# zju3dv/EnvGS

Measured on AMD Instinct MI355X. Metric: train iters/s (fwd+bwd of the render hot path + Adam step, one 800x800 view per GPU per iter) + render Mpix/s, higher is better.
Workload: dtype f32

## Files before the change

envgs_amd/_lib.py:

```python
import ctypes
import os

import torch

HERE = os.path.dirname(os.path.abspath(__file__))
LIB_PATH = os.path.join(HERE, "libenvgs_hip.so")
_lib = None

c_void_p, c_int, c_uint32, c_size_t = ctypes.c_void_p, ctypes.c_int, ctypes.c_uint32, ctypes.c_size_t


class RasterCfg(ctypes.Structure):
    _fields_ = [("P", ctypes.c_int32), ("sh_degree", ctypes.c_int32), ("sh_coeffs", ctypes.c_int32),
                ("channels", ctypes.c_int32), ("width", ctypes.c_int32), ("height", ctypes.c_int32),
                ("bg_len", ctypes.c_int32), ("debug", ctypes.c_int32), ("scale_modifier", ctypes.c_float),
                ("tanfovx", ctypes.c_float), ("tanfovy", ctypes.c_float), ("feature_f16", ctypes.c_int32)]


class AdamTensor(ctypes.Structure):
    _fields_ = [("param", ctypes.c_void_p), ("grad", ctypes.c_void_p), ("exp_avg", ctypes.c_void_p), ("exp_avg_sq", ctypes.c_void_p),
                ("numel", ctypes.c_int64), ("lr", ctypes.c_float), ("step", ctypes.c_float)]


class RowsTensor(ctypes.Structure):
# ... 8 lines not shown
    _fields_ = ([("P", ctypes.c_int64), ("N", ctypes.c_int32), ("flags", ctypes.c_uint32)]
                + [(n, ctypes.c_float) for n in ("grad_threshold", "size_limit", "split_screen_threshold", "min_opacity", "min_gradient", "r")]
                + [(n, ctypes.c_void_p) for n in ("ga", "dn", "mr", "wa", "scal", "opac", "cls", "scan", "counters", "temp")]
                + [("temp_bytes", ctypes.c_size_t)])


class DensifyRewriteArgs(ctypes.Structure):
    _fields_ = ([("P", ctypes.c_int64), ("out_rows", ctypes.c_int64), ("n_samples", ctypes.c_int64), ("N", ctypes.c_int32), ("count", ctypes.c_int32),
                 ("ratio_n", ctypes.c_double), ("r", ctypes.c_float), ("reserved0", ctypes.c_uint32)]
                + [(n, ctypes.c_void_p) for n in ("cls", "scan", "counters", "scal", "rotation", "samples")]
                + [("tensors", ctypes.POINTER(GrowTensor))])


class TraceLists(ctypes.Structure):
    _fields_ = [("hit_lists", ctypes.c_void_p), ("hit_cnt", ctypes.c_void_p), ("n_used", ctypes.c_void_p), ("cap", ctypes.c_int32),
                ("surf_acc", ctypes.c_void_p), ("surf_cnt", ctypes.c_void_p), ("surf_off", ctypes.c_void_p),
                ("scan_temp", ctypes.c_void_p), ("scan_temp_bytes", ctypes.c_size_t), ("ray_keys", ctypes.c_void_p),
                ("ray_order", ctypes.c_void_p), ("ray_sort_temp", ctypes.c_void_p), ("ray_sort_temp_bytes", ctypes.c_size_t),
                ("records", ctypes.c_void_p),
                ("num_records", ctypes.c_uint64), ("hit_state", ctypes.c_void_p), ("entries", ctypes.c_void_p), ("pairs", ctypes.c_void_p),
                ("n_entries", ctypes.c_void_p), ("compact_rows", ctypes.c_uint64), ("row_off", ctypes.c_void_p), ("batch_rows", ctypes.c_void_p),
                ("row_blk", ctypes.c_void_p), ("sh_perm", ctypes.c_void_p), ("state_planes", ctypes.c_int32),
                ("sparse_hits", ctypes.c_void_p), ("sparse_cap", ctypes.c_uint64),
                ("defer_reduce", ctypes.c_uint32), ("reserved0", ctypes.c_uint32)]


class TraceCfg(ctypes.Structure):
    _fields_ = [("P", ctypes.c_int32), ("num_rays", ctypes.c_int32), ("sh_degree", ctypes.c_int32),
                ("sh_coeffs", ctypes.c_int32), ("max_trace_depth", ctypes.c_int32), ("start_from_first", ctypes.c_int32),
                ("has_others", ctypes.c_int32), ("bg_len", ctypes.c_int32), ("debug", ctypes.c_int32),
                ("ray_h", ctypes.c_int32), ("ray_w", ctypes.c_int32),
                ("scale_modifier", ctypes.c_float), ("specular_threshold", ctypes.c_float), ("feature_f16", ctypes.c_int32)]


class SupervisorArgs(ctypes.Structure):
    _fields_ = ([("N", ctypes.c_int64), ("P", ctypes.c_int64), ("flags", ctypes.c_uint32), ("reserved0", ctypes.c_uint32),
                 ("weight", ctypes.c_float * 5), ("reserved1", ctypes.c_float)]
                + [(n, ctypes.c_void_p) for n in ("norm_map", "surf_norm_map", "acc_map", "dpt_map", "dist_map", "env_opacity", "prior", "msk", "R", "near_far")]
                + [(n, ctypes.c_int64) for n in ("norm_map_row", "norm_map_ch", "surf_norm_map_row", "surf_norm_map_ch", "acc_map_row", "dpt_map_row",
                                                 "dist_map_row", "env_opacity_row", "prior_row", "prior_ch", "msk_row")]
                + [(n, ctypes.c_void_p) for n in ("g_norm_map", "g_surf_norm_map", "g_acc_map", "g_dist_map", "g_env_opacity", "partial")])


class SurfelInputsArgs(ctypes.Structure):
    _fields_ = ([(n, ctypes.c_int32) for n in ("P", "sh_degree", "sh_coeffs", "spec_channels")]
                + [(n, ctypes.c_void_p) for n in ("xyz", "features_dc", "features_rest", "scaling", "rotation", "opacity", "specular", "roughness", "campos",
                                                  "scales", "rotations", "opacities", "specular_act", "roughness_act", "shs", "colors", "others", "vertices",
# ... 148 lines not shown
```

envgs_amd/csrc/trace_api.hip:

```cpp
#include "trace_common.h"

#include <mutex>


namespace envgs {

constexpr int MAX_SEG = 4;

static int persistent_grid(int R, int per_cu = 8)
{
    int dev = 0, cus = 256;
    if (hipGetDevice(&dev) == hipSuccess) {
        int v = 0;
        if (hipDeviceGetAttribute(&v, hipDeviceAttributeMultiprocessorCount, dev) == hipSuccess && v > 0) cus = v;
    }
    const int want = (R + 63) / 64;
    const int cap = cus * per_cu;
    return want < cap ? (want > 0 ? want : 1) : cap;
}

static int stride_grid(int R, int per_block)
{
    const int want = (R + per_block - 1) / per_block;
    const int cap = 256 * 32;
// ... 50 lines not shown
    return true;
}

static int join_deferred(hipStream_t stream)
{
    int dev = 0;
    if (hipGetDevice(&dev) != hipSuccess || dev < 0 || dev >= 16) return 0;
    std::lock_guard<std::mutex> lk(s_mu);
    if (!s_def_pending[dev]) return 0;
    s_def_pending[dev] = false;
    return hipStreamWaitEvent(stream, s_def_done[dev], 0) == hipSuccess ? 0 : ENVGS_ERR_BAD_ARG;
}

static TraceArgs base_args(const envgs_trace_cfg *cfg, const float *nodes, const float *srec, const float *shs, const float *colors_precomp,
                           const float *others_precomp, const float *bg, const float *ray_o, const float *ray_d, uint32_t *counters)
{
    TraceArgs A = TraceArgs{};
    A.P = cfg->P; A.R = cfg->num_rays; A.D = cfg->sh_degree; A.M = cfg->sh_coeffs; A.ND = 1;
    A.start_from_first = cfg->start_from_first; A.has_others = cfg->has_others; A.bg_len = cfg->bg_len; A.spec_thr = cfg->specular_threshold;
    A.nodes = (const float4 *)nodes; A.srec = (const float4 *)srec; A.shs = shs; A.colors = colors_precomp; A.others = others_precomp;
    A.bg = bg; A.ray_o = ray_o; A.ray_d = ray_d; A.counter = counters;
    A.mod = cfg->scale_modifier; A.f16 = cfg->feature_f16; A.exp = debug_switch(ENVGS_DBG_TRACE);
    return A;
}

static unsigned sparse_capacity(const envgs_trace_lists *L)
{
    return (unsigned)(L->sparse_cap > 0xFFFFFFF0ull ? 0xFFFFFFF0ull : L->sparse_cap);
}

extern "C" {

size_t envgs_trace_ray_sort_temp_bytes(int32_t num_rays) { return ray_sort_temp_bytes(num_rays); }

int envgs_trace_ray_order(int32_t num_rays, const float *ray_o, const float *ray_d, const float *nodes, int32_t P, uint64_t *pairs,
                          uint32_t *order, void *temp, size_t temp_bytes, void *stream)
{
    if (num_rays < 0 || P < 0) return ENVGS_ERR_BAD_ARG;
    if (num_rays == 0) return 0;
    if (!ray_o || !ray_d || !pairs || !order || !temp || (P > 0 && !nodes)) return ENVGS_ERR_BAD_ARG;
    return launch_ray_sort(num_rays, ray_o, ray_d, (const float4 *)nodes, P, pairs, order, temp, temp_bytes, (hipStream_t)stream);
}

int envgs_trace_forward(const envgs_trace_cfg *cfg, const float *nodes, const float *ray_o, const float *ray_d,
                        const float *means3D, const float *scales, const float *rotations, const float *opacities,
                        const float *shs, const float *colors_precomp, const float *others_precomp, const float *bg,
// ... 133 lines not shown
            }
            {
                ProfScope p2(K_TRACE_SORT, st);
                const dim3 g(stride_grid(rays_seg, 4)), b(256);
                if (S.shp) hipLaunchKernelGGL((sort_composite_fwd<4, false, true>), g, b, 0, st, S);
                else hipLaunchKernelGGL((sort_composite_fwd<4, false, false>), g, b, 0, st, S);
                if (S.cap > 256) {
                    const dim3 gl(min(stride_grid(rays_seg, 256), 512));
                    if (S.cap <= 512) { if (S.shp) hipLaunchKernelGGL((sort_composite_fwd<8, true, true>), gl, b, 0, st, S); else hipLaunchKernelGGL((sort_composite_fwd<8, true, false>), gl, b, 0, st, S); }
                    else { if (S.shp) hipLaunchKernelGGL((sort_composite_fwd<16, true, true>), gl, b, 0, st, S); else hipLaunchKernelGGL((sort_composite_fwd<16, true, false>), gl, b, 0, st, S); }
                }
            }
            ENVGS_CHECK_LAUNCH(dcfg, st);
            {
                ProfScope p8(K_TRACE_REGISTER, st);
                const dim3 gr(stride_grid(rays_seg, 64)), br(64 * RH_W);
                if (S.pairs && S.cap <= 256) hipLaunchKernelGGL(register_hits<true>, gr, br, 0, st, S);
                else hipLaunchKernelGGL(register_hits<false>, gr, br, 0, st, S);
            }
            ENVGS_CHECK_LAUNCH(dcfg, st);
        }
        for (int i = 1; i < nseg; i++)
            if (hipEventRecord(ev_join[i], aux[i]) != hipSuccess || hipStreamWaitEvent(stream, ev_join[i], 0) != hipSuccess) return ENVGS_ERR_BAD_ARG;
        hipLaunchKernelGGL(unpack_surfel_acc, dim3((cfg->P + 255) / 256), dim3(256), 0, stream, cfg->P, A.wfrac, A.surf_acc, L->surf_cnt, wet,
                           counters);
        ENVGS_CHECK_LAUNCH(dcfg, stream);
        {
            const int rc = launch_scan(L->surf_cnt, L->surf_off, cfg->P * NCOPY, L->scan_temp, L->scan_temp_bytes, stream);
            if (rc) return rc;
        }
        A.only_overflow = 1;
    } else {
        const int rcp = launch_prepare(stream);
        if (rcp) return rcp;
        ENVGS_CHECK_LAUNCH(dcfg, stream);
    }
    { ProfScope p4(K_TRACE_KBUF_FWD, stream); hipLaunchKernelGGL(trace_fwd, dim3(persistent_grid(cfg->num_rays)), dim3(64), 0, stream, A, rh, rw); }
    ENVGS_CHECK_LAUNCH(dcfg, stream);
    return 0;
}

int envgs_trace_backward(const envgs_trace_cfg *cfg, const float *nodes, const float *ray_o, const float *ray_d,
                         const float *means3D, const float *scales, const float *rotations, const float *opacities,
                         const float *shs, const float *colors_precomp, const float *others_precomp, const float *bg,
                         const float *srec, uint32_t *counters, const float *rgb, const float *dpt, const float *acc,
                         const float *norm, const float *aux, const float *final_T, const float *dL_drgb, const float *dL_ddpt,
                         const float *dL_dacc, const float *dL_dnorm, const float *dL_daux, float *geo_rec, float *dmeans3D,
                         float *dgrads3D, float *dscales, float *drots, float *dopacities, float *dshs, float *dcolors,
// ... 31 lines not shown
    A.geo_rec = geo_rec; A.dshs = dshs; A.dcolors = dcolors; A.dothers = dothers; A.dray_o = dray_o; A.dray_d = dray_d;
    if (A.exp & (8 | 16 | 512 | 2048 | 4096 | 8192)) return ENVGS_ERR_BAD_ARG;
    int rh, rw; ray_layout(cfg, &rh, &rw);
    bool deferred = false, have_records = false;
    int def_dev = 0;
    {
        ProfScope prof_(K_TRACE_BWD, stream);
        if (lists_wanted(cfg, L) && !lists_usable_bwd(cfg, L)) return ENVGS_ERR_BAD_ARG;
        if (lists_usable_bwd(cfg, L)) {
            A.hits = (uint2 *)L->hit_lists; A.hit_cnt = L->hit_cnt; A.n_used = L->n_used; A.cap = L->cap;
            if (L->ray_keys && L->ray_order && L->ray_sort_temp && !(A.exp & 64)) A.order = L->ray_order + cfg->num_rays;
            if (L->records && L->num_records > 0 && L->surf_cnt && L->surf_off && L->hit_state && L->entries && L->pairs && L->n_entries) {
                A.surf_cnt = L->surf_cnt; A.surf_off = L->surf_off; A.records = L->records; A.num_records = L->num_records;
                A.state = (float4 *)L->hit_state; A.entries = (unsigned long long *)L->entries; A.pairs = L->pairs; A.n_entries = L->n_entries;
                if (L->compact_rows > 0) {
                    if (!L->row_off || !L->batch_rows) return ENVGS_ERR_BAD_ARG;
                    A.row_off = L->row_off; A.batch_rows = (const uint2 *)L->batch_rows;
                }
                A.state_plane = L->compact_rows > 0 ? (size_t)L->compact_rows : (size_t)cfg->num_rays * (size_t)L->cap;
                {
                    ProfScope p5(K_TRACE_LIST_BWD, stream);
                    const bool rgb_only = dL_drgb && !dL_ddpt && !dL_dacc && !dL_dnorm && !dL_daux;
                    if (L->state_planes == 1 && !rgb_only) return ENVGS_ERR_BAD_ARG;
                    const dim3 g(stride_grid((cfg->num_rays + 63) / 64, 1));
                    if (rgb_only) hipLaunchKernelGGL((batch_surfel_bwd<true, false>), g, dim3(64), 0, stream, A);
                    else if (cfg->has_others) hipLaunchKernelGGL((batch_surfel_bwd<false, true>), g, dim3(64), 0, stream, A);
                    else hipLaunchKernelGGL((batch_surfel_bwd<false, false>), g, dim3(64), 0, stream, A);
                    if (L->sparse_hits && L->sparse_cap > 0) {
                        A.sparse = (uint4 *)L->sparse_hits;
                        A.sparse_cap = sparse_capacity(L);
                        hipLaunchKernelGGL(sparse_hits_bwd, dim3(2048), dim3(256), 0, stream, A, rgb_only ? 1 : 0);
                    }
                }
                have_records = true;
                if ((dflags & ENVGS_TRACE_DEFER) && aux_objects(&def_dev)) deferred = true;
                else if (!accumulate) { ProfScope p7(K_TRACE_REDUCE, stream); hipLaunchKernelGGL(reduce_surfel_records, dim3(stride_grid(cfg->P, 16)), dim3(256), 0, stream, A); }
            } else {
                if (!(L->surf_cnt && L->surf_off && L->hit_state && L->entries && L->pairs && L->n_entries) || (L->records == nullptr && L->num_records > 0))
                    return ENVGS_ERR_BAD_ARG;
            }
            A.only_overflow = 1;
        }
        if (accumulate && join_deferred(stream)) return ENVGS_ERR_BAD_ARG;
        { ProfScope p6(K_TRACE_KBUF_BWD, stream); hipLaunchKernelGGL(trace_bwd, dim3(persistent_grid(cfg->num_rays)), dim3(64), 0, stream, A, rh, rw); }
    }
    ENVGS_CHECK_LAUNCH(dcfg, stream);
    if ((dflags & ENVGS_TRACE_DEFER) && !deferred && aux_objects(&def_dev)) deferred = true;
// ... 31 lines not shown
```

envgs_amd/csrc/trace_common.h:

```cpp
#ifndef ENVGS_TRACE_COMMON_H
#define ENVGS_TRACE_COMMON_H

#include "common.h"
#include "prof.h"

#include <cstdlib>
#include <cstring>

#include "../../include/envgs_trace.h"

namespace envgs {

constexpr int KBUF = 16;
constexpr int STACK = 64;
constexpr int NCOPY = 8;
constexpr int MAX_ROUNDS = 256;
constexpr float UV_MAX = 3.0f;
constexpr int MID = ENVGS_MID_CHANNELS;
constexpr int SREC = ENVGS_SREC_STRIDE;
constexpr int NODE = ENVGS_NODE_STRIDE;

constexpr float kC0 = 0.28209479177387814f;
constexpr float kC1 = 0.4886025119029199f;
static __device__ __constant__ float tC2[5] = {1.0925484305920792f, -1.0925484305920792f, 0.31539156525252005f,
// ... 114 lines not shown
    const unsigned *surf_off;
    float *records;
    unsigned long long num_records;
    const unsigned *order;
    int exp;
    int only_overflow;
    int batch0, batch1;
    uint4 *sparse;
    unsigned sparse_cap;
    int sparse_max;
    int reduce_adds;
    int seg;
    unsigned long long *entries;
    unsigned *pairs;
    int *n_entries;
    unsigned *long_list;
    float4 *state;
    size_t state_plane;
    int colour_state;
    unsigned *batch_cnt;
    const unsigned *row_off;
    const uint2 *batch_rows;
    const void *shp;
};

struct KBuf {
    float t[KBUF];
    int id[KBUF];
    int n;
    __device__ __forceinline__ void reset() {
#pragma unroll
        for (int i = 0; i < KBUF; i++) { t[i] = 3.0e38f; id[i] = 0x7fffffff; }
        n = 0;
    }
    __device__ __forceinline__ void insert(float ct, int cid) {
#pragma unroll
        for (int i = 0; i < KBUF; i++) {
            const bool before = (ct < t[i]) || (ct == t[i] && cid < id[i]);
            const float tt = before ? t[i] : ct; const int ii = before ? id[i] : cid;
            t[i] = before ? ct : t[i]; id[i] = before ? cid : id[i];
            ct = tt; cid = ii;
        }
        n = n < KBUF ? n + 1 : KBUF;
    }
};

// ... 408 lines not shown
struct ForwardPrepare {
    ZeroBatch zero; int zero_blocks;
    int P, rec_blocks; float mod; const float *means, *scales, *rots, *opac; float *srec;
    int perm_blocks, nb, f16; const void *shs; void *shp;
};
__global__ void __launch_bounds__(256) forward_prepare(const ForwardPrepare F);
__global__ void __launch_bounds__(64) trace_fwd(const TraceArgs A, const int ray_h, const int ray_w);
__global__ void __launch_bounds__(64) trace_bwd(const TraceArgs A, const int ray_h, const int ray_w);
__global__ void __launch_bounds__(256, 8)
collect_hits_coop(const TraceArgs A, const float4 *__restrict__ nodes, const float4 *__restrict__ nodes4, const float4 *__restrict__ srec);

template <int EMAX, bool LONG, bool QSH> __global__ void __launch_bounds__(256) sort_composite_fwd(const TraceArgs A);
extern template __global__ void __launch_bounds__(256) sort_composite_fwd<4, false, false>(const TraceArgs A);
extern template __global__ void __launch_bounds__(256) sort_composite_fwd<8, true, false>(const TraceArgs A);
extern template __global__ void __launch_bounds__(256) sort_composite_fwd<16, true, false>(const TraceArgs A);
extern template __global__ void __launch_bounds__(256) sort_composite_fwd<4, false, true>(const TraceArgs A);
extern template __global__ void __launch_bounds__(256) sort_composite_fwd<8, true, true>(const TraceArgs A);
extern template __global__ void __launch_bounds__(256) sort_composite_fwd<16, true, true>(const TraceArgs A);
template <bool CACHED> __global__ void __launch_bounds__(64 * RH_W) register_hits(const TraceArgs A);
__global__ void __launch_bounds__(256) row_scan_blocks(unsigned *__restrict__ blk, int n, unsigned *rows_used, unsigned *seg_base);
__global__ void __launch_bounds__(256) row_offsets(const TraceArgs A, const unsigned *__restrict__ blk, unsigned *__restrict__ row_off, uint2 *__restrict__ batch_rows,
                                                   const unsigned *__restrict__ seg_base, unsigned long long limit);
__global__ void __launch_bounds__(256) unpack_surfel_acc(int P, int wfrac, const unsigned long long *__restrict__ acc, unsigned *__restrict__ cnt,
                                                         float *__restrict__ wet, unsigned *ray_counter);
__global__ void __launch_bounds__(256) sparse_hits_bwd(const TraceArgs A, const int rgbo);
template <bool RGBO, bool OTH> __global__ void __attribute__((amdgpu_waves_per_eu(ENVGS_BSB_WAVES, ENVGS_BSB_WAVES))) __launch_bounds__(64) batch_surfel_bwd(const TraceArgs A);
extern template __global__ void __attribute__((amdgpu_waves_per_eu(ENVGS_BSB_WAVES, ENVGS_BSB_WAVES))) __launch_bounds__(64) batch_surfel_bwd<false, false>(const TraceArgs A);
extern template __global__ void __attribute__((amdgpu_waves_per_eu(ENVGS_BSB_WAVES, ENVGS_BSB_WAVES))) __launch_bounds__(64) batch_surfel_bwd<false, true>(const TraceArgs A);
extern template __global__ void __attribute__((amdgpu_waves_per_eu(ENVGS_BSB_WAVES, ENVGS_BSB_WAVES))) __launch_bounds__(64) batch_surfel_bwd<true, false>(const TraceArgs A);
__global__ void __launch_bounds__(256) reduce_surfel_records(const TraceArgs A);
__global__ void __launch_bounds__(256) finish_surfel_grads(int P, const float *__restrict__ rots, const float *__restrict__ geo_rec,
                                                           float *__restrict__ dmeans, float *__restrict__ dscales, float *__restrict__ dopac,
                                                           float *__restrict__ drots, float *__restrict__ dgrads3D);

}
#endif
```

envgs_amd/csrc/trace_lists.hip:

```cpp
#include "trace_common.h"

#ifndef ENVGS_SCF_KO
#define ENVGS_SCF_KO 0
#endif
namespace envgs {

template <int S>
__device__ __forceinline__ unsigned xlane(unsigned v)
{
    if constexpr (S == 1) return (unsigned)__builtin_amdgcn_update_dpp(0, (int)v, 0xB1, 0xf, 0xf, true);
    else if constexpr (S == 2) return (unsigned)__builtin_amdgcn_update_dpp(0, (int)v, 0x4E, 0xf, 0xf, true);
    else if constexpr (S == 32) {
        const envgs_u2 r = __builtin_amdgcn_permlane32_swap(v, v, false, false);
        return (threadIdx.x & 32) ? r.x : r.y;
    } else return (unsigned)__builtin_amdgcn_ds_swizzle((int)v, 0x1F | (S << 10));
}

template <int E, int SIZE, int STRIDE>
__device__ __forceinline__ void bitonic_layer(unsigned long long (&k)[E], const int lane)
{
    if constexpr (STRIDE >= 64) {
        constexpr int SE = STRIDE / 64;
#pragma unroll
        for (int e = 0; e < E; e++)
// ... 628 lines not shown
    const int slot_end = min(A.R, A.batch1 * 64);
    const int slot = A.batch0 * 64 + (int)blockIdx.x * 256 + (int)threadIdx.x;
    const int lane = threadIdx.x & 63, batch = slot >> 6;
    if (batch >= A.batch1) return;
    const unsigned cnt = rows_of_slot(A, slot, slot_end);
    const float incl = wave_scan_add((float)cnt);
    const unsigned long long row0 = base + (unsigned long long)blk[batch];
    const unsigned long long row = row0 + (unsigned long long)((unsigned)incl - cnt);
    const bool fits = row + cnt <= limit;
    if (slot < slot_end) {
        row_off[slot] = (unsigned)(fits ? row : 0ull);
        if (!fits && cnt > 0u) {
            A.hit_cnt[ray_of(A, slot)] = A.cap + 1;
            atomicAdd(A.counter + 21, 1u);
        }
    }
    const unsigned tot = (unsigned)wave_bcast(incl, 63);
    if (lane == 0) {
        const unsigned long long end = row0 + tot < limit ? row0 + tot : limit;
        batch_rows[batch] = make_uint2((unsigned)(row0 < limit ? row0 : limit), (unsigned)(end > row0 ? end - row0 : 0ull));
    }
}

__global__ void __launch_bounds__(256)
unpack_surfel_acc(int P, int wfrac, const unsigned long long *__restrict__ acc, unsigned *__restrict__ cnt, float *__restrict__ wet, unsigned *ray_counter)
{
    const int i = blockIdx.x * 256 + threadIdx.x;
    if (i == 0 && ray_counter) *ray_counter = 0u;
    if (i >= P) return;
    unsigned long long wsum = 0;
#pragma unroll
    for (int c = 0; c < NCOPY; c++) {
        const unsigned long long a = acc[(size_t)i * NCOPY + c];
        cnt[(size_t)i * NCOPY + c] = (unsigned)(a & 0xFFFFFFull);
        wsum += a >> 24;
    }
    const float w = (float)((double)wsum / (double)(1ull << wfrac));
    if (w != 0.0f) wet[i] += w;
}


template __global__ void sort_composite_fwd<4, false, false>(const TraceArgs A);
template __global__ void sort_composite_fwd<8, true, false>(const TraceArgs A);
template __global__ void sort_composite_fwd<16, true, false>(const TraceArgs A);
template __global__ void sort_composite_fwd<4, false, true>(const TraceArgs A);
template __global__ void sort_composite_fwd<8, true, true>(const TraceArgs A);
template __global__ void sort_composite_fwd<16, true, true>(const TraceArgs A);

}
```

envgs_amd/csrc/trace_surfel_bwd.hip:

```cpp
#include "trace_common.h"

namespace envgs {

#define ENVGS_LDS_FENCE() do { __builtin_amdgcn_s_waitcnt(0xc07f); __builtin_amdgcn_sched_barrier(0); } while (0)
#ifndef ENVGS_BS_GROUP
#define ENVGS_BS_GROUP 15
#endif
constexpr int BS_GROUP = ENVGS_BS_GROUP;
static_assert(BS_GROUP <= 16, "stage() assigns four lanes per entry");
#ifndef ENVGS_BSB_KO
#define ENVGS_BSB_KO 0
#endif

typedef float f32x4 __attribute__((ext_vector_type(4)));
constexpr int BT_PITCH = 96;
constexpr int RECW = 64;
template <bool RGBO, bool OTH>
__global__ void __attribute__((amdgpu_waves_per_eu(ENVGS_BSB_WAVES, ENVGS_BSB_WAVES))) __launch_bounds__(64)
batch_surfel_bwd(const TraceArgs A)
{
    static_assert(!(RGBO && OTH), "the colour-only form never touches `others`");
    __shared__ float4 sdat[2][BS_GROUP][16];
    __shared__ unsigned long long sdesc[2][BS_GROUP];
    __shared__ unsigned short kmat[2][BS_GROUP][64];
    __shared__ unsigned spb[2][BS_GROUP];
    __shared__ unsigned scn[2][BS_GROUP];
    __shared__ float btile[16][BT_PITCH];
    __shared__ float2 sox[2][BS_GROUP];
    const int lane = threadIdx.x;
    const int nb = (A.D + 1) * (A.D + 1);
    const int nbatch = (A.R + 63) >> 6;
    for (int batch = blockIdx.x; batch < nbatch; batch += gridDim.x) {
        const int base = batch << 6;
        const int copy = batch & (NCOPY - 1);
        const int r = ray_of(A, base + lane);
        const bool valid = r < A.R && A.hit_cnt[r < A.R ? r : 0] <= A.cap;
        const int rr = r < A.R ? r : 0;
        float basis[16], Box, Boy, Boz, Bdx, Bdy, Bdz, gR0, gR1, gR2, gD, gA, gN0, gN1, gN2, gX0, gX1, Fsum;
        {
            BwdRay B;
            bwd_load_ray(A, rr, B);
#pragma unroll
            for (int k = 0; k < 16; k++) basis[k] = 0.f;
            sh_basis(A.D, B.ux, B.uy, B.uz, basis);
            if (A.M == 0) basis[0] = kC0;
            if (!(B.il > 0.0f && B.il < 3.0e38f)) {
#pragma unroll
                for (int k = 0; k < 16; k++) basis[k] = 0.f;
            }
            Box = B.ox; Boy = B.oy; Boz = B.oz; Bdx = B.dx; Bdy = B.dy; Bdz = B.dz;
            gR0 = B.gR0; gR1 = B.gR1; gR2 = B.gR2;
            if constexpr (RGBO) { gD = gA = gN0 = gN1 = gN2 = gX0 = gX1 = 0.f; }
            else { gD = B.gD; gA = B.gA; gN0 = B.gN0; gN1 = B.gN1; gN2 = B.gN2; gX0 = B.gX0; gX1 = B.gX1; }
            Fsum = bwd_final_dot(B);
        }
// ... 497 lines not shown
```

envgs_amd/tracing.py:

```python
from typing import NamedTuple

import torch
from torch import nn

from . import _lib


class SurfelTracingSettings(NamedTuple):
    image_height: int
    image_width: int
    tanfovx: float
    tanfovy: float
    bg: torch.Tensor
    scale_modifier: float
    viewmatrix: torch.Tensor
    projmatrix: torch.Tensor
    sh_degree: int
    campos: torch.Tensor
    prefiltered: bool
    debug: bool
    max_trace_depth: int
    specular_threshold: float


# ... 123 lines not shown
    if n * item <= (32 << 20):
        return torch.empty(shape, dtype=dtype, device=dev)
    k = max(n - 1, 1).bit_length() - 1
    for q in (5, 6, 7, 8):
        if (q << k) >> 2 >= n:
            return torch.empty((q << k) >> 2, dtype=dtype, device=dev)[:n].view(shape)
    raise AssertionError


def _carve_i32(dev, sizes):
    offs, total = {}, 0
    for k, n in sizes.items():
        offs[k] = total
        total += ((int(n) + 63) // 64) * 64
    buf = torch.empty(max(total, 64), dtype=torch.int32, device=dev)
    out = {k: buf[o:o + int(sizes[k])] for k, o in offs.items()}
    out["_i32_block"] = buf
    return out


SPARSE = {"mode": "auto", "below": 6.0, "cap": None, "poison": None}
QUAD_SH = {"on": True}
KEEP_LISTS = {"on": False}


_DEFERRED = {"pending": False, "keep": None, "dev": None}


def join_deferred_gradients():
    if not _DEFERRED["pending"]:
        return
    dev = _DEFERRED["dev"]
    with torch.cuda.device(dev):
        _lib.check(_lib.load().envgs_trace_backward_join(_stream(dev)), "envgs_trace_backward_join")
    _DEFERRED.update(pending=False, keep=None, dev=None)


class _DeferBarrier(torch.autograd.Function):

    @staticmethod
    def forward(ctx, *ts):
        return tuple(t.view_as(t) for t in ts)

    @staticmethod
    def backward(ctx, *gs):
        join_deferred_gradients()
# ... 48 lines not shown
    from .raster import _featc
    shs = _featc(shs); colors_precomp = _featc(colors_precomp); others_precomp = _f32c(others_precomp)
    f16 = any(t is not None and t.dtype == torch.float16 for t in (shs, colors_precomp))
    bg = _f32c(settings.bg).reshape(-1).to(dev)
    cfg = _cfg(settings, P, R, shs, others_precomp, start_from_first, lead, f16)
    ND = cfg.max_trace_depth + 1
    f32 = dict(dtype=torch.float32, device=dev)
    srec = torch.empty(max(P, 1), 16, **f32)
    counters = torch.empty(96, dtype=torch.int32, device=dev)
    rgb = torch.empty(R, 3, **f32); dpt = torch.empty(R, 1, **f32); acc = torch.empty(R, 1, **f32)
    norm = torch.empty(R, 3, **f32); dist = torch.empty(R, 1, **f32); aux = torch.empty(R, 2, **f32)
    mid = torch.empty(R, 16 * ND, **f32); wet = torch.empty(P, 1, **f32); final_T = torch.empty(R, **f32)
    cap = caps.next_cap(dev) if (use_lists and ND == 1 and P > 0 and R > 0) else 0
    rows = 0
    lists = None
    keep = {}
    if cap:
        i32 = dict(dtype=torch.int32, device=dev)
        sb = lib.envgs_raster_scan_temp_bytes(NCOPY * P)
        rb = lib.envgs_trace_ray_sort_temp_bytes(R)
        nbatch = (R + 63) // 64
        keep = _carve_i32(dev, dict(hit_cnt=R, n_used=R, surf_acc=2 * P * NCOPY, surf_cnt=P * NCOPY,
                                    surf_off=P * NCOPY, scan_temp=(max(sb, 1) + 3) // 4, ray_keys=2 * R, ray_order=2 * R, ray_sort_temp=(max(rb, 1) + 3) // 4,
                                    n_entries=2 * nbatch, row_off=R, batch_rows=2 * nbatch, row_blk=nbatch + 16))
        keep["n_entries"] = keep["n_entries"].view(nbatch, 2)
        keep["hit_lists"] = _scratch((R, cap, 2), torch.int32, dev)
        srt = SORT_RAYS["on"]
        if shs is not None and shs.shape[1] == 16 and QUAD_SH["on"]:
            keep["sh_perm"] = torch.empty(P, 48, dtype=shs.dtype, device=dev)
        if need_grad:
            colour_only = bool(getattr(caps, "colour_only", False))
            sw = 4 if colour_only else (10 if others_precomp is not None else 8)
            if COMPACT["on"] and srt:
                rows = caps.next_rows(R, cap)
                keep.update(hit_state=_scratch((rows, sw), torch.float32, dev), entries=_scratch((rows,), torch.int64, dev), pairs=_scratch((rows,), torch.int32, dev))
            else:
                keep.update(hit_state=_scratch((R, cap, sw), torch.float32, dev), entries=_scratch((nbatch, 64 * cap), torch.int64, dev),
                            pairs=_scratch((nbatch, 64 * cap), torch.int32, dev))
        sparse = SPARSE["mode"] == "on" or (SPARSE["mode"] == "auto" and caps.hits_per_entry is not None and caps.hits_per_entry < SPARSE["below"])
        if "hit_state" in keep and sparse:
            n_rows = rows if rows else R * cap
            keep["sparse_hits"] = _scratch((max(4096, n_rows), 4), torch.int32, dev)
            if SPARSE.get("poison") is not None:
                keep["sparse_hits"].fill_(int(SPARSE["poison"]))
        sparse_cap = 0
        if "sparse_hits" in keep:
            sparse_cap = keep["sparse_hits"].shape[0] if SPARSE.get("cap") is None else min(int(SPARSE["cap"]), keep["sparse_hits"].shape[0])
        lists = _lib.TraceLists(keep["hit_lists"].data_ptr(), keep["hit_cnt"].data_ptr(), keep["n_used"].data_ptr(), cap,
                                keep["surf_acc"].data_ptr(), keep["surf_cnt"].data_ptr(), keep["surf_off"].data_ptr(),
                                keep["scan_temp"].data_ptr(), sb, keep["ray_keys"].data_ptr() if srt else None,
                                keep["ray_order"].data_ptr() if srt else None, keep["ray_sort_temp"].data_ptr() if srt else None, rb, None, 0,
                                *[(keep[k].data_ptr() if k in keep else None) for k in ("hit_state", "entries", "pairs")],
                                keep["n_entries"].data_ptr() if "hit_state" in keep else None, rows,
                                *[(keep[k].data_ptr() if (k in keep and rows) else None) for k in ("row_off", "batch_rows", "row_blk")],
                                keep["sh_perm"].data_ptr() if "sh_perm" in keep else None, 0,
                                keep["sparse_hits"].data_ptr() if "sparse_hits" in keep else None, sparse_cap)
        if "hit_state" in keep and getattr(caps, "colour_only", False):
            lists.state_planes = 1
            keep["colour_only"] = True
        if "hit_state" in keep and getattr(caps, "defer_reduce", False):
            keep["defer_reduce"] = True
    p = _lib.ptr
    _lib.check(lib.envgs_trace_forward(cfg, p(nodes), p(ro), p(rd), p(means3D), p(scales), p(rotations), p(opacities), p(shs),
                                       p(colors_precomp), p(others_precomp), p(bg), p(srec), p(counters), p(rgb), p(dpt), p(acc),
                                       p(norm), p(dist), p(aux), p(mid), p(wet), p(final_T), lists, _stream(dev)), "envgs_trace_forward")
    LAST_STATS.update(P=P, R=R, caps=caps, rows=rows, counters=counters, n_entries=(keep.get("n_entries") if "hit_state" in keep else None), cap=cap,
                      lists=((keep["hit_lists"], keep["n_used"], keep["hit_cnt"]) if (cap and KEEP_LISTS["on"]) else None),
                      records=(dict(sparse_hits=keep.get("sparse_hits"), sparse_cap=sparse_cap, entries=keep["entries"], pairs=keep["pairs"],
                                    n_entries=keep["n_entries"], batch_rows=(keep["batch_rows"].view(-1, 2) if rows else None),
                                    ray_order=(keep["ray_order"][R:] if SORT_RAYS["on"] else None), surf_cnt=keep["surf_cnt"], surf_off=keep["surf_off"])
                               if (cap and KEEP_LISTS["on"] and "hit_state" in keep) else None))
    if cap:
        if "hit_state" in keep and not KEEP_LISTS["on"]:
            keep.pop("hit_lists")
            lists.hit_lists = None
        caps.publish(counters, dev, rays=R)
        if "hit_state" in keep:
            keep["n_rec_host"], keep["n_rec_claim"] = caps.pinned_word()
            keep["n_rec_host"].copy_(keep["surf_off"].view(-1)[NCOPY * P - 1:NCOPY * P], non_blocking=True)
            keep["n_rec_event"] = torch.cuda.Event(); keep["n_rec_event"].record(torch.cuda.current_stream(dev))
    saved = dict(cfg=cfg, nodes=nodes, ro=ro, rd=rd, means3D=means3D, scales=scales, rotations=rotations, opacities=opacities,
                 shs=shs, colors_precomp=colors_precomp, others=others_precomp, bg=bg, srec=srec, counters=counters,
                 rgb=(rgb if ND == 1 else mid[:, 13:16].contiguous()),
                 dpt=dpt, acc=acc, norm=norm, aux=aux, final_T=final_T, lead=lead, lists=lists, keep=keep, cap=cap)
    outs = (rgb.reshape(lead + (3,)), dpt.reshape(lead + (1,)), acc.reshape(lead + (1,)), norm.reshape(lead + (3,)),
            dist.reshape(lead + (1,)), aux.reshape(lead + (2,)), mid.reshape(lead + (16 * ND,)), wet)
    return outs, saved


class _BounceChain:

    def __init__(self):
        self.acc = None
# ... 397 lines not shown
```

include/envgs_raster.h:

```cpp
#ifndef ENVGS_RASTER_H
#define ENVGS_RASTER_H

#include <stddef.h>
#include <stdint.h>

#ifdef __cplusplus
extern "C" {
#endif

#if defined(__GNUC__)
#define ENVGS_API __attribute__((visibility("default")))
#else
#define ENVGS_API
#endif

#define ENVGS_TILE 16
#define ENVGS_GEOM_STRIDE 16
#define ENVGS_GRAD_STRIDE 32

typedef enum envgs_status {
    ENVGS_OK = 0,
    ENVGS_ERR_BAD_ARG = -1,
    ENVGS_ERR_TEMP_TOO_SMALL = -2
} envgs_status;
// ... 41 lines not shown
                          const uint32_t *point_list, const uint32_t *ranges,
                          const float *final_T, const int32_t *n_contrib, const uint8_t *contrib_mask ,
                          const float *dL_dcolor, const float *dL_dallmap,
                          const float *means3D, const float *scales, const float *rotations,
                          const float *shs, const uint8_t *clamped, const float *transmat_precomp,
                          const int32_t *radii,
                          const float *viewmatrix, const float *projmatrix, const float *campos,
                          float *grad_rec,
                          float *dmeans3D, float *dmeans2D, float *dscales, float *drots,
                          float *dshs, float *dcolors, float *dopacities, float *dtransmat_precomp,
                          void *stream);

ENVGS_API void envgs_prof_enable(int on);
ENVGS_API void envgs_prof_select(uint64_t kernel_mask);
ENVGS_API int envgs_prof_read(int kernel_id, double *total_ms, int *launches);
ENVGS_API const char *envgs_prof_kernel_name(int kernel_id);

#define ENVGS_DBG_TRACE 0
#define ENVGS_DBG_SEGMENTS 1
#define ENVGS_DBG_COLLECT_WGS 2
#define ENVGS_DBG_RASTER_EXACT 3
#define ENVGS_DBG_RAYKEY 4
#define ENVGS_DBG_SPARSE 5
#define ENVGS_DBG_COUNT 6
ENVGS_API void envgs_debug_set(int32_t which, int32_t value);
ENVGS_API int32_t envgs_debug_get(int32_t which);

#ifdef __cplusplus
}
#endif
#endif
```

include/envgs_trace.h:

```cpp
#ifndef ENVGS_TRACE_H
#define ENVGS_TRACE_H

#include <stddef.h>
#include <stdint.h>

#include "envgs_raster.h"

#ifdef __cplusplus
extern "C" {
#endif

#define ENVGS_NODE_STRIDE 16
#define ENVGS_SREC_STRIDE 16
#define ENVGS_GEOREC_STRIDE 16
#define ENVGS_MID_CHANNELS 16
#define ENVGS_WIDE_EMPTY ((int32_t)0x80000000)

typedef struct envgs_trace_cfg {
    int32_t P;
    int32_t num_rays;
    int32_t sh_degree;
    int32_t sh_coeffs;
    int32_t max_trace_depth;
    int32_t start_from_first;
// ... 16 lines not shown
    uint32_t *surf_off;
    void *scan_temp;
    size_t scan_temp_bytes;
    uint32_t *ray_keys;
    uint32_t *ray_order;
    void *ray_sort_temp;
    size_t ray_sort_temp_bytes;
    float *records;
    uint64_t num_records;
    float *hit_state;
    uint64_t *entries;
    uint32_t *pairs;
    int32_t *n_entries;
    uint64_t compact_rows;
    uint32_t *row_off;
    uint32_t *batch_rows;
    uint32_t *row_blk;
    void *sh_perm;
    int32_t state_planes;
    uint32_t *sparse_hits;
    uint64_t sparse_cap;
    uint32_t defer_reduce;
    uint32_t reserved0;
} envgs_trace_lists;
#define ENVGS_TRACE_DEFER 1u
#define ENVGS_TRACE_ACCUMULATE 2u
#define ENVGS_TRACE_NO_FINISH 4u

ENVGS_API size_t envgs_bvh_temp_bytes(int32_t P);
ENVGS_API size_t envgs_bvh_node_floats(int32_t P);

ENVGS_API int envgs_bvh_build(int32_t P, const float *vertices, const float *opacities, float *nodes, void *temp, size_t temp_bytes,
                              int32_t debug, void *stream);

ENVGS_API int envgs_bvh_refit(int32_t P, const float *vertices, const float *opacities, const float *nodes_prev, float *nodes, void *temp,
                              size_t temp_bytes, int32_t debug, void *stream);

ENVGS_API int envgs_bvh_quality(int32_t P, const float *nodes, float *out2, void *stream);

ENVGS_API size_t envgs_trace_ray_sort_temp_bytes(int32_t num_rays);
ENVGS_API int envgs_trace_ray_order(int32_t num_rays, const float *ray_o, const float *ray_d, const float *nodes, int32_t P,
                                    uint64_t *pairs, uint32_t *order, void *temp, size_t temp_bytes, void *stream);
ENVGS_API int envgs_trace_forward(const envgs_trace_cfg *cfg, const float *nodes,
                                  const float *ray_o, const float *ray_d,
                                  const float *means3D, const float *scales, const float *rotations, const float *opacities,
                                  const float *shs, const float *colors_precomp, const float *others_precomp, const float *bg,
                                  float *srec, uint32_t *counters,
// ... 24 lines not shown
```

Baseline: 136.2.

## Schedule surfel backward batches in descending-cost order for load balance

Adds a single-block pass, folded into the unpack_surfel_acc launch, that bins 64-ray batches by entry count into 32 cost classes. It writes a permutation ordering the heaviest batches first. The tracer backward then launches one workgroup per batch in that order instead of a strided persistent grid, aiming to cut tail imbalance across CUs. The cost is an extra serial one-block pass on the stream, a larger grid, and the loss of the strided coherence ordering.

```diff
diff --git a/envgs_amd/_lib.py b/envgs_amd/_lib.py
--- a/envgs_amd/_lib.py
+++ b/envgs_amd/_lib.py
@@ -54,7 +54,7 @@
                 ("n_entries", ctypes.c_void_p), ("compact_rows", ctypes.c_uint64), ("row_off", ctypes.c_void_p), ("batch_rows", ctypes.c_void_p),
                 ("row_blk", ctypes.c_void_p), ("sh_perm", ctypes.c_void_p), ("state_planes", ctypes.c_int32),
                 ("sparse_hits", ctypes.c_void_p), ("sparse_cap", ctypes.c_uint64),
-                ("defer_reduce", ctypes.c_uint32), ("reserved0", ctypes.c_uint32)]
+                ("defer_reduce", ctypes.c_uint32), ("reserved0", ctypes.c_uint32), ("bwd_order", ctypes.c_void_p)]
 
 
 class TraceCfg(ctypes.Structure):
diff --git a/envgs_amd/csrc/trace_api.hip b/envgs_amd/csrc/trace_api.hip
--- a/envgs_amd/csrc/trace_api.hip
+++ b/envgs_amd/csrc/trace_api.hip
@@ -96,6 +96,12 @@
     A.bg = bg; A.ray_o = ray_o; A.ray_d = ray_d; A.counter = counters;
     A.mod = cfg->scale_modifier; A.f16 = cfg->feature_f16; A.exp = debug_switch(ENVGS_DBG_TRACE);
     return A;
+}
+
+static int bwd_order_classes()
+{
+    const int k = debug_switch(ENVGS_DBG_BALANCE) >> 8;
+    return k > 0 ? k : ENVGS_BWD_ORDER_CLASSES;
 }
 
 static unsigned sparse_capacity(const envgs_trace_lists *L)
@@ -275,8 +281,9 @@
         }
         for (int i = 1; i < nseg; i++)
             if (hipEventRecord(ev_join[i], aux[i]) != hipSuccess || hipStreamWaitEvent(stream, ev_join[i], 0) != hipSuccess) return ENVGS_ERR_BAD_ARG;
-        hipLaunchKernelGGL(unpack_surfel_acc, dim3((cfg->P + 255) / 256), dim3(256), 0, stream, cfg->P, A.wfrac, A.surf_acc, L->surf_cnt, wet,
-                           counters);
+        unsigned *bwd_order = (L->bwd_order && L->n_entries && L->entries && L->pairs && L->hit_state) ? L->bwd_order : nullptr;
+        hipLaunchKernelGGL(unpack_surfel_acc, dim3((cfg->P + 255) / 256 + (bwd_order ? 1 : 0)), dim3(256), 0, stream, cfg->P, A.wfrac, A.surf_acc, L->surf_cnt, wet,
+                           counters, (const int *)L->n_entries, nbatch_all, bwd_order, bwd_order_classes());
         ENVGS_CHECK_LAUNCH(dcfg, stream);
         {
             const int rc = launch_scan(L->surf_cnt, L->surf_off, cfg->P * NCOPY, L->scan_temp, L->scan_temp_bytes, stream);
@@ -354,7 +361,9 @@
                     ProfScope p5(K_TRACE_LIST_BWD, stream);
                     const bool rgb_only = dL_drgb && !dL_ddpt && !dL_dacc && !dL_dnorm && !dL_daux;
                     if (L->state_planes == 1 && !rgb_only) return ENVGS_ERR_BAD_ARG;
-                    const dim3 g(stride_grid((cfg->num_rays + 63) / 64, 1));
+                    const bool by_cost = L->bwd_order && !(debug_switch(ENVGS_DBG_BALANCE) & 1);
+                    A.bwd_order = by_cost ? L->bwd_order : nullptr;
+                    const dim3 g(by_cost ? (cfg->num_rays + 63) / 64 : stride_grid((cfg->num_rays + 63) / 64, 1));
                     if (rgb_only) hipLaunchKernelGGL((batch_surfel_bwd<true, false>), g, dim3(64), 0, stream, A);
                     else if (cfg->has_others) hipLaunchKernelGGL((batch_surfel_bwd<false, true>), g, dim3(64), 0, stream, A);
                     else hipLaunchKernelGGL((batch_surfel_bwd<false, false>), g, dim3(64), 0, stream, A);
diff --git a/envgs_amd/csrc/trace_common.h b/envgs_amd/csrc/trace_common.h
--- a/envgs_amd/csrc/trace_common.h
+++ b/envgs_amd/csrc/trace_common.h
@@ -160,6 +160,7 @@
     const unsigned *row_off;
     const uint2 *batch_rows;
     const void *shp;
+    const unsigned *bwd_order;
 };
 
 struct KBuf {
@@ -614,7 +615,8 @@
 __global__ void __launch_bounds__(256) row_offsets(const TraceArgs A, const unsigned *__restrict__ blk, unsigned *__restrict__ row_off, uint2 *__restrict__ batch_rows,
                                                    const unsigned *__restrict__ seg_base, unsigned long long limit);
 __global__ void __launch_bounds__(256) unpack_surfel_acc(int P, int wfrac, const unsigned long long *__restrict__ acc, unsigned *__restrict__ cnt,
-                                                         float *__restrict__ wet, unsigned *ray_counter);
+                                                         float *__restrict__ wet, unsigned *ray_counter, const int *__restrict__ n_entries, int nbatch,
+                                                         unsigned *__restrict__ bwd_order, int order_classes);
 __global__ void __launch_bounds__(256) sparse_hits_bwd(const TraceArgs A, const int rgbo);
 template <bool RGBO, bool OTH> __global__ void __attribute__((amdgpu_waves_per_eu(ENVGS_BSB_WAVES, ENVGS_BSB_WAVES))) __launch_bounds__(64) batch_surfel_bwd(const TraceArgs A);
 extern template __global__ void __attribute__((amdgpu_waves_per_eu(ENVGS_BSB_WAVES, ENVGS_BSB_WAVES))) __launch_bounds__(64) batch_surfel_bwd<false, false>(const TraceArgs A);
diff --git a/envgs_amd/csrc/trace_lists.hip b/envgs_amd/csrc/trace_lists.hip
--- a/envgs_amd/csrc/trace_lists.hip
+++ b/envgs_amd/csrc/trace_lists.hip
@@ -674,10 +674,79 @@
     }
 }
 
+constexpr int ORDER_MAX_CLASSES = 1024;
+constexpr int ORDER_SEGS = 4;
+__device__ __forceinline__ int order_count(const int *__restrict__ n_entries, int b)
+{
+    const int c = n_entries[2 * b] + n_entries[2 * b + 1];
+    return c < 0 ? 0 : (c > (1 << 20) ? (1 << 20) : c);
+}
+__device__ __forceinline__ int order_bin(int cnt, int maxc, int K)
+{
+    cnt = cnt > maxc ? maxc : cnt;
+    return K - 1 - (int)(((unsigned)cnt * (unsigned)K) / ((unsigned)maxc + 1u));
+}
+__device__ void build_bwd_order(const int *__restrict__ n_entries, const int nbatch, unsigned *__restrict__ order, int K)
+{
+    __shared__ unsigned s_off[ORDER_MAX_CLASSES * ORDER_SEGS];
+    __shared__ int s_max;
+    K = K < 1 ? 1 : (K > ORDER_MAX_CLASSES ? ORDER_MAX_CLASSES : K);
+    const int tid = threadIdx.x, lane = tid & 63, wave = tid >> 6;
+    const int seglen = (((nbatch + ORDER_SEGS - 1) / ORDER_SEGS) + 63) & ~63;
+    if (tid == 0) s_max = 0;
+    for (int i = tid; i < K * ORDER_SEGS; i += 256) s_off[i] = 0u;
+    __syncthreads();
+    int m = 0;
+#pragma unroll 8
+    for (int b = tid; b < nbatch; b += 256) m = max(m, order_count(n_entries, b));
+    if (m > 0) atomicMax(&s_max, m);
+    __syncthreads();
+    const int maxc = s_max;
+#pragma unroll 8
+    for (int b = tid; b < nbatch; b += 256) atomicAdd(&s_off[order_bin(order_count(n_entries, b), maxc, K) * ORDER_SEGS + b / seglen], 1u);
+    __syncthreads();
+    if (wave == 0) {
+        unsigned carry = 0u;
+        for (int k0 = 0; k0 < K * ORDER_SEGS; k0 += 64) {
+            const unsigned v = s_off[k0 + lane];
+            unsigned incl = v;
+#pragma unroll
+            for (int d = 1; d < 64; d <<= 1) { const unsigned o = __shfl_up(incl, d); if (lane >= d) incl += o; }
+            s_off[k0 + lane] = carry + incl - v;
+            carry += __shfl(incl, 63);
+        }
+    }
+    __syncthreads();
+    int nbits = 0;
+    while ((1 << nbits) < K) nbits++;
+    const int seg0 = wave * seglen, seg1 = min(seg0 + seglen, nbatch);
+    int next = seg0 + lane < seg1 ? order_count(n_entries, seg0 + lane) : 0;
+    for (int b0 = seg0; b0 < seg1; b0 += 64) {
+        const int b = b0 + lane;
+        const bool act = b < seg1;
+        const int cnt = next;
+        next = b + 64 < seg1 ? order_count(n_entries, b + 64) : 0;
+        const int bin = act ? order_bin(cnt, maxc, K) : 0;
+        unsigned long long mask = __ballot(act);
+        for (int bit = 0; bit < nbits; bit++) {
+            const bool one = (bin >> bit) & 1;
+            const unsigned long long bb = __ballot(act && one);
+            mask &= one ? bb : ~bb;
+        }
+        const int rank = __popcll(mask & ((1ull << lane) - 1ull));
+        unsigned first = 0u;
+        if (act && rank == 0) first = atomicAdd(&s_off[bin * ORDER_SEGS + wave], (unsigned)__popcll(mask));
+        first = __shfl(first, act ? __ffsll((long long)mask) - 1 : lane);
+        if (act && first + (unsigned)rank < (unsigned)nbatch) order[first + (unsigned)rank] = (unsigned)b;
+    }
+}
+
 __global__ void __launch_bounds__(256)
-unpack_surfel_acc(int P, int wfrac, const unsigned long long *__restrict__ acc, unsigned *__restrict__ cnt, float *__restrict__ wet, unsigned *ray_counter)
-{
-    const int i = blockIdx.x * 256 + threadIdx.x;
+unpack_surfel_acc(int P, int wfrac, const unsigned long long *__restrict__ acc, unsigned *__restrict__ cnt, float *__restrict__ wet, unsigned *ray_counter,
+                  const int *__restrict__ n_entries, int nbatch, unsigned *__restrict__ bwd_order, int order_classes)
+{
+    if (bwd_order && blockIdx.x == 0) { build_bwd_order(n_entries, nbatch, bwd_order, order_classes); return; }
+    const int i = (int)(blockIdx.x - (bwd_order ? 1u : 0u)) * 256 + threadIdx.x;
     if (i == 0 && ray_counter) *ray_counter = 0u;
     if (i >= P) return;
     unsigned long long wsum = 0;
diff --git a/envgs_amd/csrc/trace_surfel_bwd.hip b/envgs_amd/csrc/trace_surfel_bwd.hip
--- a/envgs_amd/csrc/trace_surfel_bwd.hip
+++ b/envgs_amd/csrc/trace_surfel_bwd.hip
@@ -30,7 +30,9 @@
     const int lane = threadIdx.x;
     const int nb = (A.D + 1) * (A.D + 1);
     const int nbatch = (A.R + 63) >> 6;
-    for (int batch = blockIdx.x; batch < nbatch; batch += gridDim.x) {
+    for (int slot = blockIdx.x; slot < nbatch; slot += gridDim.x) {
+        const int batch = A.bwd_order ? (int)A.bwd_order[slot] : slot;
+        if ((unsigned)batch >= (unsigned)nbatch) continue;
         const int base = batch << 6;
         const int copy = batch & (NCOPY - 1);
         const int r = ray_of(A, base + lane);
diff --git a/envgs_amd/tracing.py b/envgs_amd/tracing.py
--- a/envgs_amd/tracing.py
+++ b/envgs_amd/tracing.py
@@ -169,6 +169,12 @@
 SPARSE = {"mode": "auto", "below": 6.0, "cap": None, "poison": None}
 QUAD_SH = {"on": True}
 KEEP_LISTS = {"on": False}
+BWD_ORDER = {"on": True}
+BWD_ORDER_CLASSES = 32
+
+
+def bwd_order_class(counts, classes=BWD_ORDER_CLASSES):
+    return (counts * int(classes)) // (int(counts.max()) + 1)
 
 
 _DEFERRED = {"pending": False, "keep": None, "dev": None}
@@ -263,7 +269,7 @@
         nbatch = (R + 63) // 64
         keep = _carve_i32(dev, dict(hit_cnt=R, n_used=R, surf_acc=2 * P * NCOPY, surf_cnt=P * NCOPY,
                                     surf_off=P * NCOPY, scan_temp=(max(sb, 1) + 3) // 4, ray_keys=2 * R, ray_order=2 * R, ray_sort_temp=(max(rb, 1) + 3) // 4,
-                                    n_entries=2 * nbatch, row_off=R, batch_rows=2 * nbatch, row_blk=nbatch + 16))
+                                    n_entries=2 * nbatch, row_off=R, batch_rows=2 * nbatch, row_blk=nbatch + 16, bwd_order=nbatch))
         keep["n_entries"] = keep["n_entries"].view(nbatch, 2)
         keep["hit_lists"] = _scratch((R, cap, 2), torch.int32, dev)
         srt = SORT_RAYS["on"]
@@ -296,6 +302,8 @@
                                 *[(keep[k].data_ptr() if (k in keep and rows) else None) for k in ("row_off", "batch_rows", "row_blk")],
                                 keep["sh_perm"].data_ptr() if "sh_perm" in keep else None, 0,
                                 keep["sparse_hits"].data_ptr() if "sparse_hits" in keep else None, sparse_cap)
+        if "hit_state" in keep and BWD_ORDER["on"]:
+            lists.bwd_order = keep["bwd_order"].data_ptr()
         if "hit_state" in keep and getattr(caps, "colour_only", False):
             lists.state_planes = 1
             keep["colour_only"] = True
@@ -309,7 +317,8 @@
                       lists=((keep["hit_lists"], keep["n_used"], keep["hit_cnt"]) if (cap and KEEP_LISTS["on"]) else None),
                       records=(dict(sparse_hits=keep.get("sparse_hits"), sparse_cap=sparse_cap, entries=keep["entries"], pairs=keep["pairs"],
                                     n_entries=keep["n_entries"], batch_rows=(keep["batch_rows"].view(-1, 2) if rows else None),
-                                    ray_order=(keep["ray_order"][R:] if SORT_RAYS["on"] else None), surf_cnt=keep["surf_cnt"], surf_off=keep["surf_off"])
+                                    ray_order=(keep["ray_order"][R:] if SORT_RAYS["on"] else None), surf_cnt=keep["surf_cnt"], surf_off=keep["surf_off"],
+                                    bwd_order=(keep["bwd_order"] if BWD_ORDER["on"] else None))
                                if (cap and KEEP_LISTS["on"] and "hit_state" in keep) else None))
     if cap:
         if "hit_state" in keep and not KEEP_LISTS["on"]:
diff --git a/include/envgs_raster.h b/include/envgs_raster.h
--- a/include/envgs_raster.h
+++ b/include/envgs_raster.h
@@ -87,7 +87,8 @@
 #define ENVGS_DBG_RASTER_EXACT 3
 #define ENVGS_DBG_RAYKEY 4
 #define ENVGS_DBG_SPARSE 5
-#define ENVGS_DBG_COUNT 6
+#define ENVGS_DBG_BALANCE 6
+#define ENVGS_DBG_COUNT 7
 ENVGS_API void envgs_debug_set(int32_t which, int32_t value);
 ENVGS_API int32_t envgs_debug_get(int32_t which);
 
diff --git a/include/envgs_trace.h b/include/envgs_trace.h
--- a/include/envgs_trace.h
+++ b/include/envgs_trace.h
@@ -62,7 +62,9 @@
     uint64_t sparse_cap;
     uint32_t defer_reduce;
     uint32_t reserved0;
+    uint32_t *bwd_order;
 } envgs_trace_lists;
+#define ENVGS_BWD_ORDER_CLASSES 32
 #define ENVGS_TRACE_DEFER 1u
 #define ENVGS_TRACE_ACCUMULATE 2u
 #define ENVGS_TRACE_NO_FINISH 4u
diff --git a/profiles/balance_profile.py b/profiles/balance_profile.py
--- /dev/null
+++ b/profiles/balance_profile.py
@@ -0,0 +1,92 @@
+import argparse
+import importlib
+import importlib.util
+import os
+import sys
+
+HERE = os.path.dirname(os.path.abspath(__file__))
+sys.path[:] = [os.path.dirname(HERE)] + [p for p in sys.path if os.path.abspath(p or ".") != HERE]
+
+import numpy as np
+import torch
+
+_spec = importlib.util.spec_from_file_location("sched_model", os.path.join(HERE, "sched_model.py"))
+sched_model = importlib.util.module_from_spec(_spec)
+_spec.loader.exec_module(sched_model)
+from envgs_amd import envgs_step, raster, synth, tracing
+
+
+def main():
+    ap = argparse.ArgumentParser()
+    ap.add_argument("--out", required=True)
+    ap.add_argument("--save-counts", default=None, help="directory for the per-view count arrays (.npy)")
+    ap.add_argument("--gaussians", type=int, default=300000)
+    ap.add_argument("--env-gaussians", type=int, default=163840)
+    ap.add_argument("--res", type=int, default=800)
+    a = ap.parse_args()
+    dev = torch.device("cuda:0")
+    P, H, W, C = a.gaussians, a.res, a.res, 5
+    g = synth.base_gaussians(P, seed=0, device=dev)
+    ge = synth.env_gaussians(a.env_gaussians, seed=1, device=dev)
+    cams = [synth.orbit_camera(v, n_views=8, H=H, W=W, fx=1111.1 * W / 800.0, device=dev) for v in range(8)]
+    names = ["means3D", "shs", "opacities", "scales", "rotations"]
+    params = {k: g[k].clone().requires_grad_(True) for k in names}
+    params["specular"] = g["specular"].repeat(1, C - 4).contiguous().clone().requires_grad_(True)
+    params["roughness"] = g["roughness"].clone().requires_grad_(True)
+    env = {k: ge[k].clone().requires_grad_(True) for k in names}
+    pkg = importlib.import_module("diff_surfel_rasterization_wet_ch05")
+    import diff_surfel_tracing as tpkg
+    envgs_step.FUSED["on"] = True
+    tracer = tpkg.SurfelTracer()
+    bg = torch.zeros(3, device=dev)
+    sh_degree = torch.tensor([3], device=dev)
+    lines = []
+    out = lambda s="": (lines.append(s), print(s, flush=True))
+    out("balance of the coarse work, %d base / %d environment surfels, %dx%d, the eight bench views" % (P, a.env_gaussians, H, W))
+    out()
+    out("== tracer backward: entries per 64-ray batch of the environment trace ==")
+    for v, cam in enumerate(cams):
+        for _ in range(2):
+            envgs_step.envgs_forward(pkg, tpkg, tracer, cam, synth.get_rays(cam), params, env, bg, bg, sh_degree)
+        torch.cuda.synchronize()
+        tracing.join_deferred_gradients()
+        ne = tracing.LAST_STATS["n_entries"].cpu().numpy().astype(np.int64)
+        if a.save_counts:
+            os.makedirs(a.save_counts, exist_ok=True)
+            np.save(os.path.join(a.save_counts, "n_entries_view%d.npy" % v), ne)
+        out("view %d" % v)
+        out(sched_model.format_report(sched_model.report(ne)).rstrip("\n"))
+    out()
+    out("== raster: per-tile work summed over the eight XCD bands of xcd_tile() ==")
+    out("(instances = entries of the tile's list; contributing = entries some pixel of the tile blended; passes = (8x8 quadrant, splat) passes of R7)")
+    for v, cam in enumerate(cams):
+        st = pkg.GaussianRasterizationSettings(image_height=H, image_width=W, tanfovx=cam.tanfovx, tanfovy=cam.tanfovy, bg=torch.zeros(C, device=dev),
+                                               scale_modifier=1.0, viewmatrix=cam.world_view_transform, projmatrix=cam.full_proj_transform,
+                                               sh_degree=sh_degree, campos=cam.camera_center, prefiltered=False, debug=False)
+        with torch.no_grad():
+            _, sv = raster.rasterize_forward(C, g["means3D"], None, torch.zeros(P, C, device=dev), g["opacities"], g["scales"], g["rotations"], None, st)
+        rg = sv["ranges"].view(-1, 2).long().cpu().numpy()
+        cm = sv["contrib_mask"][:sv["N"]].cpu().numpy()
+        inst = rg[:, 1] - rg[:, 0]
+        c_con = np.concatenate([[0], np.cumsum(cm != 0)])
+        c_pas = np.concatenate([[0], np.cumsum(np.unpackbits(cm[:, None], axis=1)[:, 4:].sum(1))])
+        con = c_con[rg[:, 1]] - c_con[rg[:, 0]]
+        pas = c_pas[rg[:, 1]] - c_pas[rg[:, 0]]
+        ntiles = len(inst)
+        per = (ntiles + 7) // 8
+        if a.save_counts:
+            np.save(os.path.join(a.save_counts, "tiles_view%d.npy" % v), np.stack([inst, con, pas], 1))
+        out("view %d: %d tiles, %d instances, %d contributing, %d passes" % (v, ntiles, inst.sum(), con.sum(), pas.sum()))
+        for name, arr in (("instances", inst), ("contributing", con), ("passes", pas)):
+            bands = np.array([arr[x * per:(x + 1) * per].sum() for x in range(8)], dtype=np.float64)
+            nz = arr[arr > 0]
+            out("    %-12s band / mean: %s   max / mean %.3f   per tile: mean %.0f  p50 %.0f  p90 %.0f  max %d" % (
+                name, " ".join("%.2f" % (b / bands.mean()) for b in bands), bands.max() / bands.mean(), arr.mean(),
+                np.percentile(nz, 50) if nz.size else 0, np.percentile(nz, 90) if nz.size else 0, arr.max()))
+    os.makedirs(os.path.dirname(os.path.abspath(a.out)), exist_ok=True)
+    with open(a.out, "w") as f:
+        f.write("\n".join(lines) + "\n")
+
+
+if __name__ == "__main__":
+    main()
diff --git a/profiles/sched_model.py b/profiles/sched_model.py
--- /dev/null
+++ b/profiles/sched_model.py
@@ -0,0 +1,74 @@
+import argparse
+import heapq
+import os
+import sys
+
+if __name__ == "__main__":
+    sys.path[:] = [p for p in sys.path if os.path.abspath(p or ".") != os.path.dirname(os.path.abspath(__file__))]
+
+import numpy as np
+
+
+def makespan(workgroup_costs, slots=2048, xcds=8):
+    per = max(1, slots // xcds)
+    end = 0.0
+    for x in range(xcds):
+        mine = workgroup_costs[x::xcds]
+        free = [0.0] * per
+        heapq.heapify(free)
+        for c in mine:
+            t = heapq.heappop(free) + float(c)
+            heapq.heappush(free, t)
+            end = max(end, t)
+    return end
+
+
+def ideal(costs, slots=2048):
+    costs = np.asarray(costs, dtype=np.float64)
+    return max(costs.sum() / slots, costs.max() if costs.size else 0.0)
+
+
+def strided_workgroups(costs, grid=8192):
+    costs = np.asarray(costs, dtype=np.float64)
+    g = min(grid, len(costs))
+    out = np.zeros(g)
+    for s in range(0, len(costs), g):
+        part = costs[s:s + g]
+        out[:len(part)] += part
+    return out
+
+
+def class_order(counts, classes):
+    counts = np.asarray(counts, dtype=np.int64)
+    key = counts if classes <= 0 else (counts * classes) // (int(counts.max()) + 1)
+    return np.argsort(-key, kind="stable")
+
+
+def report(counts, slots=2048, fixed=0.0):
+    counts = np.asarray(counts, dtype=np.int64)
+    if counts.ndim == 2:
+        counts = counts.sum(1)
+    cost = counts.astype(np.float64) + fixed
+    lo = ideal(cost, slots)
+    rows = [("coherence order, 8192 workgroups (round 6)", makespan(strided_workgroups(cost), slots) / lo)]
+    for k in (1, 8, 32, 0):
+        rows.append(("one workgroup per batch, %s" % ("full sort" if k == 0 else "K = %d" % k), makespan(cost[class_order(counts, k)], slots) / lo))
+    return dict(batches=int(counts.size), mean=float(counts.mean()), cv=float(counts.std() / max(counts.mean(), 1e-9)), max=int(counts.max()),
+                min=int(counts.min()), rounds=float(counts.size / slots), rows=rows)
+
+
+def format_report(r):
+    s = "batches %d  entries per batch: mean %.1f  cv %.3f  min %d  max %d  (%.2f rounds of the resident slots)\n" % (
+        r["batches"], r["mean"], r["cv"], r["min"], r["max"], r["rounds"])
+    for name, v in r["rows"]:
+        s += "    %-46s makespan / ideal %.3f\n" % (name, v)
+    return s
+
+
+if __name__ == "__main__":
+    ap = argparse.ArgumentParser()
+    ap.add_argument("counts")
+    ap.add_argument("--slots", type=int, default=2048, help="resident workgroups: 256 CUs x 4 SIMDs x 2 wavefronts")
+    ap.add_argument("--fixed", type=float, default=0.0, help="cost of a batch beyond its entries, in entries")
+    a = ap.parse_args()
+    print(format_report(report(np.load(a.counts), a.slots, a.fixed)), end="")
```

New measurement: 140.7 (median of 6 runs). +3.3%, better.
